# Chuanming-Liu/DAzimSurfTomo

Measured on AMD Instinct MI355X. Metric: FMM traveltime fields/sec (256^2 grid, 16 periods) + LSQR SpMV HBM GB/s, higher is better.
Workload: dtype f32

## Files before the change

### dazimsurftomo_amd/csrc/rays.hip

```cpp
#include <cmath>
#include <chrono>
#include <unistd.h>

#include "dazim_internal.h"

#include <rocprim/device/device_scan.hpp>
#include <rocprim/device/device_radix_sort.hpp>

namespace {

#ifdef DZ_RAYS_MARK
#define RAYS_MARK(i) asm volatile("; MARK " #i ::: "memory")
#else
#define RAYS_MARK(i)
#endif

constexpr int GDX = 5, GDZ = 5;
constexpr int RM = DAZIM_RMAX;
constexpr float EARTH = 6371.0f;
constexpr float FTOL = 1e-4f;

struct RayArgs {
  dazim_geom g;
  int nx, ny, nz, kmax;
  long nray;
  const int *field;
  const float *rcx, *rcz;
  const float *scx, *scz;
  const int *period;
  const int *kidx;
  const float *veln;
  const float *ttn;
  const int *tslot;
  int tsh;
  long fstride;
  const int *fdone;
  int *defer_mark;
  int max_quads;
  int sweeps;
  const float *ttnr;
  const int *nstsr;
  const dazim_refbox *boxes;
  const float *vels;
  const double *svs, *svp, *srho;
  unsigned nvx_magic;
  const double *skern;
  const float *lsen;
  double r_dnx, r_dnz, r_dnxr, r_dnzr, r_dvx, r_dvz, r_e2dnx, r_e2dnxr;
  float dplh;
  float *dsurf;
  int *status;
  int *rbflag;
  long *count;
  int *nlist;
  unsigned short *lcell;
  float *lval;
  float *fdm_scratch;
  int LK;
  int lcap;
  const unsigned *perm;
  unsigned *qcount;
  float2 *pts;
  int *npts;
  int pcap;
  int dense;
  long *countd;
  int plain_step;
  int keep_small;
  const long *rowptr;
  float *val;
  int *col;
};

__device__ __forceinline__ float dz_sinf(float x) {
  if (!(x > 0.0f && x < 3.1415927f)) return (float)sin((double)x);
  const double y = (double)x - 1.5707963267948966192;
  const double y2 = y * y;
  double p = -1.5619206968586226e-16;
  p = fma(p, y2, 4.7794773323873853e-14);
  p = fma(p, y2, -1.1470745597729725e-11);
  p = fma(p, y2, 2.0876756987868099e-09);
  p = fma(p, y2, -2.7557319223985891e-07);
  p = fma(p, y2, 2.4801587301587302e-05);
  p = fma(p, y2, -1.3888888888888889e-03);
  p = fma(p, y2, 4.1666666666666664e-02);
  p = fma(p, y2, -0.5);
  p = fma(p, y2, 1.0);
  return (float)p;
}

__device__ __forceinline__ void step_azimuth(float x0, float z0, float x1, float z1, float &c2psi, float &s2psi) {
  const float PI_F = 3.1415926535898f;
  const float evtlat = (PI_F / 2 - x0) * 180.0f / PI_F, evtlon = z0 * 180.0f / PI_F;
  const float stalat = (PI_F / 2 - x1) * 180.0f / PI_F, stalon = z1 * 180.0f / PI_F;
  const double pi = (double)3.1415926535898f;
  const float piby2 = (float)(pi / (double)2.f);
  const double rad = (double)2.f * pi / (double)360.f;
  const double sph = (double)(1.0f / 298.257f);
  const double scolat = (double)piby2 - atan((1. - sph) * (1. - sph) * tan((double)stalat * rad));
  const double ecolat = (double)piby2 - atan((1. - sph) * (1. - sph) * tan((double)evtlat * rad));
  const double slon = (double)stalon * rad, elon = (double)evtlon * rad;
  const double a = sin(scolat) * cos(slon), b = sin(scolat) * sin(slon), c = cos(scolat);
  const double dd = sin(elon), ee = -cos(elon), cc = cos(ecolat);
  const double gg = -cc * ee, hh = cc * dd, kk = -sin(ecolat);
  const double rhs1 = (a - dd) * (a - dd) + (b - ee) * (b - ee) + c * c - (double)2.f;
  const double rhs2 = (a - gg) * (a - gg) + (b - hh) * (b - hh) + (c - kk) * (c - kk) - (double)2.f;
  double daz = atan2(rhs1, rhs2);
  if (daz < 0.0) daz = daz + 2 * pi;
  float az = (float)(daz / rad);
  if (fabsf(az - 360.f) < .00001f) az = 0.0f;
  const float rgpsi = az / 180 * PI_F;
  c2psi = (float)cos((double)(2.0f * rgpsi));
  s2psi = (float)sin((double)(2.0f * rgpsi));
}

__device__ __forceinline__ float divr(float x, double rd) { return (float)((double)x * rd); }

__device__ __forceinline__ void basis(float v, float b[4]) {
  const float om = 1.0f - v;
  b[0] = om * om * om / 6.0f;
  b[1] = (4.0f - 6.0f * (v * v) + 3.0f * (v * v * v)) / 6.0f;
  b[2] = (1.0f + 3.0f * v + 3.0f * (v * v) - 3.0f * (v * v * v)) / 6.0f;
  b[3] = v * v * v / 6.0f;
}

__device__ __forceinline__ float div6(float x) { return divr(x, 1.0 / 6.0); }
__device__ __forceinline__ float basis1(float v, int i) {
  const float w = i == 0 ? 1.0f - v : v;
  const float t2 = w * w, t3 = t2 * w;
  const float p = i == 1 ? 4.0f : 1.0f + 3.0f * v;
  const float c = i == 1 ? -6.0f : 3.0f, d = i == 1 ? 3.0f : -3.0f;
  const float n = (p + c * t2) + d * t3;
  return div6((i == 0 || i == 3) ? t3 : n);
}

__device__ __forceinline__ float vel_at(const dazim_geom &g, const float *veln, int ipx, int ipz, float drx, float drz,
                                        double rdnx, double rdnz) {
  float vel = 0.0f;
#pragma unroll
  for (int l = 1; l <= 2; l++)
#pragma unroll
    for (int m = 1; m <= 2; m++) {
      float produ = (1.0f - fabsf(divr((float)(m - 1) * g.dnz - drz, rdnz)));
      produ = produ * (1.0f - fabsf(divr((float)(l - 1) * g.dnx - drx, rdnx)));
      if (ipz - 1 + m <= g.nnz && ipx - 1 + l <= g.nnx && ipz - 1 + m >= 1 && ipx - 1 + l >= 1)
        vel = vel + veln[(size_t)(ipx - 2 + l) * g.nnz + (ipz - 2 + m)] * produ;
    }
  return vel;
}
__device__ __forceinline__ float vel_at_interior(const dazim_geom &g, const float *veln, int ipx, int ipz, float drx, float drz,
                                                 double rdnx, double rdnz) {
  float vel = 0.0f;
#pragma unroll
  for (int l = 1; l <= 2; l++)
// ... 50 lines not shown
__device__ __forceinline__ void cbar() { asm volatile("" ::: "memory"); }

template <bool EMIT, bool AZIM, bool TILED, bool MAP>
__global__ __launch_bounds__(64, AZIM ? 2 : RAYS_MINW) void rays_kernel(RayArgs A_) {
  using ArgP = const __attribute__((address_space(4))) RayArgs *;
  auto launder = [](ArgP p) {
    int z;
    asm volatile("v_mov_b32 %0, 0" : "=v"(z));
    return (ArgP)((const __attribute__((address_space(4))) char *)p + __builtin_amdgcn_readfirstlane(z));
  };
  ArgP Ap = launder((ArgP)__builtin_amdgcn_kernarg_segment_ptr());
#define A (*Ap)
#define RAYS_ARGS_FRESH Ap = launder(Ap)
  constexpr int GP = EMIT ? GP_EMIT : GP_COUNT;
  constexpr int RPW = 64 / GP;
  constexpr int LPR = 16 / GP;
  constexpr int LSTEP = 4 / LPR;
  constexpr unsigned GMASK = (1u << GP) - 1u;
  extern __shared__ __attribute__((aligned(16))) unsigned short s_lists[];
  dazim_geom g;
  g.nvx = A.g.nvx; g.nvz = A.g.nvz; g.nnx = A.g.nnx; g.nnz = A.g.nnz;
  g.gox = A.g.gox; g.goz = A.g.goz; g.dnx = A.g.dnx; g.dnz = A.g.dnz; g.dvx = A.g.dvx; g.dvz = A.g.dvz;
  const int lane = threadIdx.x, grp = lane / GP, gl = lane & (GP - 1);
  const int lm = gl & 3, l0 = gl >> 2;
  const int nnx = g.nnx, nnz = g.nnz, nvx = g.nvx, nvz = g.nvz;
  const int ldf = nvx + 2, nf = ldf * (nvz + 2);
  constexpr int NG = AZIM ? 3 : 1;
  const unsigned nvx_magic = A.nvx_magic;
  const int LC = A.lcap;
  unsigned short *s_list = s_lists + (size_t)grp * LC;
  float *gfdm = A.fdm_scratch + ((size_t)blockIdx.x * RPW + grp) * nf * NG;
  float *gfdmc = gfdm + nf, *gfdms = gfdm + 2 * nf;
  __shared__ int s_rngs[RPW][4];
  int *s_rng = s_rngs[grp];
  constexpr int RC = 8;
  const float gox = g.gox, goz = g.goz, dnx = g.dnx, dnz = g.dnz, dvx = g.dvx, dvz = g.dvz;
  const double rdnx = A.r_dnx, rdnz = A.r_dnz, rdnxr = A.r_dnxr, rdnzr = A.r_dnzr, rdvx = A.r_dvx, rdvz = A.r_dvz;
  const unsigned gmask_shift = grp * GP;
  const long nquad = (A.nray + RPW - 1) / RPW;
  const int nxcd = (gridDim.x % 8 == 0) ? 8 : 1;
  unsigned *qcnt = A.qcount + (EMIT ? 8 : 0);
  int chunk = (int)(blockIdx.x % nxcd);
  int traced = 0;
  for (;;) {
    RAYS_ARGS_FRESH;
    long quad = -1;
    if (lane == 0) {
      for (int tried = 0; tried < nxcd; tried++) {
        const long lo = nquad * chunk / nxcd, hi = nquad * (chunk + 1) / nxcd;
        const long b = lo < hi ? (long)atomicAdd(&qcnt[chunk], 1u) : hi;
        if (lo + b < hi) {
          quad = lo + b;
          break;
        }
        if (!EMIT && A.sweeps > 1 && lo < hi && b < (hi - lo) * A.sweeps) {
          quad = lo + b % (hi - lo);
          break;
        }
        chunk = (chunk + 1) % nxcd;
      }
    }
    quad = ((long)__shfl((int)(quad >> 32), 0) << 32) | (unsigned)__shfl((int)quad, 0);
    chunk = __shfl(chunk, 0);
    if (quad < 0) break;
    const long slot = quad * RPW + grp;
    if (!EMIT && A.defer_mark) {
      if (!A.defer_mark[quad]) continue;
      if (A.fdone) {
        const int fq = slot < A.nray ? A.field[A.perm ? (long)A.perm[slot] : slot] : -1;
        const int st = fq >= 0 ? __hip_atomic_load(A.fdone + fq, __ATOMIC_ACQUIRE, __HIP_MEMORY_SCOPE_AGENT) : 1;
        if (__ballot(st != 1) != 0) continue;
        __builtin_amdgcn_fence(__ATOMIC_ACQUIRE, "agent");
      }
      if (A.max_quads > 0 && traced >= A.max_quads) break;
      int mine = 0;
      if (lane == 0) mine = __hip_atomic_exchange(A.defer_mark + quad, 0, __ATOMIC_RELAXED, __HIP_MEMORY_SCOPE_AGENT);
      mine = __shfl(mine, 0);
      if (!mine) continue;
      traced++;
      if (lane == 0) atomicAdd(&A.qcount[18], 1u);
    }
    if (slot >= A.nray) continue;
    const long ray = A.perm ? (long)A.perm[slot] : slot;
    const int f = A.field[ray];
    const float scx = A.scx[f], scz = A.scz[f], rcx = A.rcx[ray], rcz = A.rcz[ray];
    const float *veln = A.veln + (size_t)(A.period[f] - 1) * nnx * nnz;
    const float *ttn = TILED ? A.ttn + (size_t)(A.tslot ? A.tslot[f] : f) * A.fstride : A.ttn + (size_t)f * nnx * nnz;
    const int tsh = TILED ? A.tsh : 0;
    auto tnode = [&](int x0, int z0) -> float {
      return TILED ? ttn[dz_tile_x(x0, tsh) + dz_tile_z(z0)] : ttn[(size_t)x0 * nnz + z0];
    };
    const float *ttnr = A.ttnr + (size_t)f * RM * RM;
    const int *nstsr = A.nstsr + (size_t)f * RM * RM;
    const dazim_refbox bx = A.boxes[f];
    const int saved = EMIT ? A.nlist[ray] : -1;
    if (saved < 0 && gl < 4) s_rng[gl] = gl < 2 ? 0x7fffffff : -1;
    cbar();
    int status = 0, rb = 0;
    if (!EMIT) {
      int irx = (int)divr(rcx - gox, rdnx) + 1, irz = (int)divr(rcz - goz, rdnz) + 1;
      if (irx < 1 || irx > nnx || irz < 1 || irz > nnz) status = DAZIM_E_RECEIVER_OUTSIDE;
      if (!status) {
        if (irx == nnx) irx--;
        if (irz == nnz) irz--;
        const int isx = (int)divr(scx - gox, rdnx) + 1, isz = (int)divr(scz - goz, rdnz) + 1;
        float sred = ((scx - rcx) * EARTH) * ((scx - rcx) * EARTH);
        const float e2 = (scz - rcz) * EARTH * dz_sinf(rcx);
        sred = sqrtf(sred + e2 * e2);
        bool sw = sred < A.dplh;
        if (isx == irx && isz == irz) sw = true;
        float trr;
        if (sw) {
          const float vs = bilin_cell(g, veln, isx, isz, scx, scz, rdnx, rdnz);
          const float vr = bilin_cell(g, veln, irx, irz, rcx, rcz, rdnx, rdnz);
          trr = 2.0f * sred / (vs + vr);
        } else {
          const float drx = (rcx - gox) - (float)(irx - 1) * dnx;
          const float drz = (rcz - goz) - (float)(irz - 1) * dnz;
          trr = 0.0f;
#pragma unroll
          for (int k = 1; k <= 2; k++)
#pragma unroll
            for (int l = 1; l <= 2; l++) {
              const float produ = (1.0f - fabsf(divr((float)(l - 1) * dnz - drz, rdnz))) *
                                  (1.0f - fabsf(divr((float)(k - 1) * dnx - drx, rdnx)));
              trr = trr + tnode(irx - 2 + k, irz - 2 + l) * produ;
            }
        }
        if (gl == 0) A.dsurf[ray] = trr;
      }
    }
    const float goxr = bx.goxr, gozr = bx.gozr, dnxr = bx.dnxr, dnzr = bx.dnzr;
    const int nnxr = bx.nnxr, nnzr = bx.nnzr;
    const int isx = (int)divr(scx - goxr, rdnxr) + 1, isz = (int)divr(scz - gozr, rdnzr) + 1;
    const float dpl = 0.5f * A.dplh;
    int ipx = (int)divr(rcx - gox, rdnx) + 1, ipz = (int)divr(rcz - goz, rdnz) + 1;
    if (ipx < 1 || ipx >= nnx || ipz < 1 || ipz >= nnz) status = DAZIM_E_RECEIVER_OUTSIDE;
    if (!status && saved < 0) {
      float x0 = rcx, z0 = rcz;
      float sinx0 = dz_sinf(x0);
      int sw = 0;
      float sred = ((scx - x0) * EARTH) * ((scx - x0) * EARTH);
      float e2 = (scz - z0) * EARTH * sinx0;
      sred = sqrtf(sred + e2 * e2);
      if (sred < 2.0f * dpl) sw = 1;
      int ipxr = (int)divr(rcx - goxr, rdnxr) + 1, ipzr = (int)divr(rcz - gozr, rdnzr) + 1;
      auto in_refined = [&](int px, int pz) -> int {
        if (px < 1 || px >= nnxr || pz < 1 || pz >= nnzr) return 0;
        const int *sp = nstsr + (size_t)(px - 1) * RM + (pz - 1);
        if (sp[0] != 0 || sp[1] != 0) return 0;
        if (sp[RM] != 0 || sp[RM + 1] != 0) return 0;
        return 1;
      };
      int igref = in_refined(ipxr, ipzr);
      if (sw == 0 && igref == 1 && ipxr == isx && ipzr == isz) sw = 1;
      const bool keep_pts = !EMIT && A.pts != nullptr && gl == 0;
      float2 *rp = A.pts ? A.pts + (size_t)ray * A.pcap : nullptr;
      int np = 1;
      if (keep_pts) {
        rp[0] = make_float2(rcx, rcz);
        if (sw == 1) { if (A.pcap > 1) rp[1] = make_float2(scx, scz); np = 2; }
      }
      int cbx = -100, cbz = -100;
      float acc[LPR], accc[LPR], accs[LPR];
#pragma unroll
      for (int q = 0; q < LPR; q++) acc[q] = accc[q] = accs[q] = 0.0f;
// ... 351 lines not shown
          float rowv = 0.0f;
          int nn = 0;
          bool cell = li < ntot;
          int c = 0;
          if (cell) c = lovf ? li : s_list[li];
          const int jj = (int)__umulhi((unsigned)c, nvx_magic) + 1, kk = c - (jj - 1) * nvx + 1;
          if (cell && lovf) cell = fabsf(gfdm[jj * ldf + kk]) >= FTOL;
          if (cell && MAP) {
            rowv = (blk == 0 ? gfdm : (blk == 1 ? gfdmc : gfdms))[jj * ldf + kk];
            keep = A.keep_small ? (rowv != 0.0f) : (fabsf(rowv) > FTOL);
            nn = blk * bstride + poff + (jj - 1) * nvx + kk;
          } else if (cell) {
            const size_t si = ((size_t)(k - 1) * A.kmax + kslot) * ncol + (size_t)jj * (nvx + 2) + kk;
            if (blk == 0) {
              const float fd = gfdm[jj * ldf + kk];
              double r;
              if (A.skern) {
                r = A.skern[si] * (double)fd;
              } else {
                const float v = A.vels[((size_t)(k - 1) * A.ny + jj) * A.nx + kk];
                const float coe_a = (2.0947f - 0.8206f * 2 * v + 0.2683f * 3 * (v * v) - 0.0251f * 4 * (v * v * v));
                const float vpft = 0.9409f + 2.0947f * v - 0.8206f * (v * v) + 0.2683f * (v * v * v) - 0.0251f * (v * v * v * v);
                const float coe_rho = coe_a * (1.6612f - 0.4721f * 2 * vpft + 0.0671f * 3 * (vpft * vpft) -
                                               0.0043f * 4 * (vpft * vpft * vpft) + 0.000106f * 5 * (vpft * vpft * vpft * vpft));
                r = (A.svp[si] * (double)coe_a + A.srho[si] * (double)coe_rho + A.svs[si]) * (double)fd;
              }
              rowv = (float)r;
              if (A.dense) {
                const float vL = A.vels[((size_t)(k - 1) * A.ny + jjL) * A.nx + kkL];
                const float caL = (2.0947f - 0.8206f * 2 * vL + 0.2683f * 3 * (vL * vL) - 0.0251f * 4 * (vL * vL * vL));
                const float vpL = 0.9409f + 2.0947f * vL - 0.8206f * (vL * vL) + 0.2683f * (vL * vL * vL) - 0.0251f * (vL * vL * vL * vL);
                const float crL = caL * (1.6612f - 0.4721f * 2 * vpL + 0.0671f * 3 * (vpL * vpL) -
                                         0.0043f * 4 * (vpL * vpL * vpL) + 0.000106f * 5 * (vpL * vpL * vpL * vpL));
                const double rd = (A.svp[si] * (double)caL + A.srho[si] * (double)crL + A.svs[si]) * (double)fd;
                keepd = (float)rd != 0.0f;
                if (EMIT && A.dense == 1) rowv = (float)rd;
              }
            } else {
              rowv = A.lsen[si] * (blk == 1 ? gfdmc : gfdms)[jj * ldf + kk];
              keepd = rowv != 0.0f;
            }
            keep = A.keep_small ? (rowv != 0.0f) : (fabsf(rowv) > FTOL);
            if (EMIT && A.dense == 1) keep = keepd;
            nn = blk * bstride + (k - 1) * nvz * nvx + (jj - 1) * nvx + kk;
          }
          if (!EMIT && A.dense == 2) cntd += __popc((unsigned)((__ballot(keepd) >> gmask_shift) & GMASK));
          const unsigned m = (unsigned)((__ballot(keep) >> gmask_shift) & GMASK);
          if (EMIT && keep) {
            const long pos = rstart + cnt + __popc(m & ((1u << gl) - 1u));
            A.val[pos] = rowv;
            A.col[pos] = nn - 1;
          }
          cnt += __popc(m);
        }
      }
    cbar();
    if (saved < 0) {
      const int x0 = max(s_rng[0], 0), x1 = min(s_rng[2] + 3, nvx + 1), z0 = max(s_rng[1], 0), z1 = min(s_rng[3] + 3, nvz + 1);
      for (int z = z0; z <= z1; z++)
        for (int x = x0 + gl; x <= x1; x += GP) {
          gfdm[z * ldf + x] = 0.0f;
          if (AZIM) { gfdmc[z * ldf + x] = 0.0f; gfdms[z * ldf + x] = 0.0f; }
        }
    } else if (!rowcache) {
      for (int i = gl; i < nlist; i += GP) {
        const int c = s_list[i];
        const int jj = (int)__umulhi((unsigned)c, nvx_magic) + 1, kk = c - (jj - 1) * nvx + 1;
        gfdm[jj * ldf + kk] = 0.0f;
        if (AZIM) { gfdmc[jj * ldf + kk] = 0.0f; gfdms[jj * ldf + kk] = 0.0f; }
      }
    }
    cbar();
    if (!EMIT && gl == 0) {
      A.count[ray] = cnt;
      if (A.dense == 2) A.countd[ray] = cntd;
      if (lovf) atomicAdd(&A.qcount[16], 1u);
      if (!status && nlist > A.LK) atomicAdd(&A.qcount[17], 1u);
    }
  }
}
#undef A
#undef RAYS_ARGS_FRESH

struct RayBuild {
  dazim_ctx *ctx;
  int nx = 0, ny = 0, nz = 0, kmax = 0, nfield = 0;
  float goxd = 0, gozd = 0, dvxd = 0, dvzd = 0;
  const float *vels = nullptr, *scx = nullptr, *scz = nullptr, *veln = nullptr, *ttn = nullptr, *ttnr = nullptr, *rcx = nullptr, *rcz = nullptr;
  const float *lsen = nullptr;
  const int *period = nullptr, *kidx = nullptr, *nstsr = nullptr, *field = nullptr;
  const dazim_refbox *boxes = nullptr;
  const double *svs = nullptr, *svp = nullptr, *srho = nullptr;
  int64_t nray = 0;
  float *dsurf = nullptr;
  dazim_csr **G = nullptr;
  int64_t *nnz_out = nullptr;
  int *n_boundary = nullptr;
  bool map = false, azim = false;
  struct StreamSwap {
    dazim_ctx *c; hipStream_t main; bool on = false;
    void restore() { if (on) { c->stream = main; on = false; } }
    ~StreamSwap() {
      if (on) (void)hipStreamSynchronize(c->stream);
      restore();
    }
  } swap;
  struct {
    DzBuf<float> vels, scx, scz, veln, ttn, ttnr, rcx, rcz, dsurf, lsen;
    DzBuf<int> period, kidx, nstsr, field;
    DzBuf<dazim_refbox> boxes;
    DzBuf<double> svs, svp, srho;
  } d;
  struct Arrays {
    dazim_ctx *c; int64_t *rp = nullptr; float *v = nullptr; int *cl = nullptr; int64_t nnz = 0, cap_nnz = 0; bool keep = false;
    ~Arrays() { if (!keep) { dz_big_put(c, rp); dz_big_put(c, v); dz_big_put(c, cl); } }
  } arrays, arrays_d;
  dazim_geom g;
  bool joint = false, tiled = false, overlap = false, twin = false;
  size_t nn = 0, nr = 0, ncol = 0, nk = 0, nr1 = 0, lds = 0;
  int64_t res_rows = 0, res_nnz = 0;
  long nwg = 0;
  double overlap_tail_s = 0.0;
  RayArgs A;
  explicit RayBuild(dazim_ctx *c) : ctx(c), swap{c, c ? c->stream : nullptr}, arrays{c}, arrays_d{c} {}
  int check() {
    if (!ctx || !G) return DAZIM_E_BAD_ARG;
    joint = map ? azim : lsen != nullptr;
    if (map) nz = 2;
    if (map && dz_opt(ctx, "rays.dense_twin", 0) != 0)
      return dz_fail(ctx, DAZIM_E_BAD_ARG, "dazim_rays_build_G_maps: option rays.dense_twin serves the 3-D program's diagnostics only");
    if (dazim_geometry(nx, ny, goxd, gozd, dvxd, dvzd, &g)) return dz_fail(ctx, DAZIM_E_BAD_ARG, "bad grid");
    if (nray < 0 || nfield < 1 || nz < 2 || kmax < 1 || (size_t)g.nvx * g.nvz > 65535u) return dz_fail(ctx, DAZIM_E_BAD_ARG, "bad arguments to dazim_rays_build_G");
    tiled = ttn == nullptr;
    if (tiled && (!ctx->fields.tiled || ctx->fields.nfield != nfield || ctx->fields.nnx != g.nnx || ctx->fields.nnz != g.nnz))
      return dz_fail(ctx, DAZIM_E_BAD_ARG, "dazim_rays_build_G: ttn is NULL and the last dazim_fmm_batch call did not keep %d fields of this grid inside the library (call it with ttn = NULL)", nfield);
    if (!scx || !scz || !period || !veln || !ttnr || !nstsr || !boxes || !dsurf ||
        (!map && (!vels || !svs || !svp || !srho)) || (nray > 0 && (!field || !rcx || !rcz)))
      return dz_fail(ctx, DAZIM_E_BAD_ARG, "dazim_rays_build_G: NULL array (the refined fields ttnr, nstsr and boxes of dazim_fmm_batch are required)");
    DZ_HIP(hipSetDevice(ctx->device));
    return 0;
  }
  int decide_overlap() {
    overlap = (bool)ctx->fmm_finish && tiled && ctx->fields.fdone && nray > 0;
    if (overlap && ctx->aux_epilogue && ctx->comm && ((DzComm *)ctx->comm)->nccl) overlap = false;
    if (overlap)
      for (const void *q : {(const void *)vels, (const void *)scx, (const void *)scz, (const void *)period, (const void *)veln,
                            (const void *)ttnr, (const void *)nstsr, (const void *)boxes, (const void *)field, (const void *)rcx,
                            (const void *)rcz, (const void *)svs, (const void *)svp, (const void *)srho, (const void *)dsurf,
                            (const void *)kidx, (const void *)lsen})
        if (q && !dz_is_device_ptr(q)) overlap = false;
    if (!overlap) { const int rcf = dz_fmm_finish(ctx); if (rcf) return rcf; }
    if (overlap) {
      DZ_HIP(hipStreamWaitEvent(ctx->stream3, ctx->ev_pre, 0));
      ctx->stream = ctx->stream3;
      swap.on = true;
    }
    return dz_join_aux(ctx);
  }
  int stage_inputs() {
    nn = (size_t)g.nnx * g.nnz; nr = (size_t)RM * RM; ncol = (size_t)nx * ny;
    int rc;
    if (!map && (rc = d.vels.init(ctx, vels, (size_t)nz * ncol, true, false))) return rc;
    if ((rc = d.scx.init(ctx, scx, nfield, true, false)) || (rc = d.scz.init(ctx, scz, nfield, true, false)) ||
        (rc = d.period.init(ctx, period, nfield, true, false)) || (rc = d.kidx.init(ctx, kidx ? kidx : period, nfield, true, false)) ||
        (rc = d.veln.init(ctx, veln, nn * kmax, true, false)) || (!tiled && (rc = d.ttn.init(ctx, ttn, nn * nfield, true, false))) ||
        (rc = d.ttnr.init(ctx, ttnr, nr * nfield, true, false)) || (rc = d.nstsr.init(ctx, nstsr, nr * nfield, true, false)) ||
        (rc = d.boxes.init(ctx, boxes, nfield, true, false)) || (rc = d.field.init(ctx, field, nray, true, false)) ||
        (rc = d.rcx.init(ctx, rcx, nray, true, false)) || (rc = d.rcz.init(ctx, rcz, nray, true, false)))
      return rc;
    nk = (size_t)nz * kmax * ncol;
    if (!map && ((rc = d.svs.init(ctx, svs, nk, true, false)) || (rc = d.svp.init(ctx, svp, nk, true, false)) ||
                  (rc = d.srho.init(ctx, srho, nk, true, false))))
      return rc;
    if ((rc = d.dsurf.init(ctx, dsurf, nray, false, true))) return rc;
    if (joint && !map && (rc = d.lsen.init(ctx, lsen, (size_t)(nz - 1) * kmax * ncol, true, false))) return rc;
    if ((rc = dz_check_range(ctx, d.period.dev, nfield, 1, kmax, "period_idx"))) return rc;
    if ((rc = dz_check_range(ctx, d.kidx.dev, nfield, 1, kmax, "kernel_idx"))) return rc;
    return dz_check_range(ctx, d.field.dev, nray, 0, nfield - 1, "field_of_ray");
  }
  int kernel_constants() {
    int rc;
    A.g = g;
    A.nx = nx; A.ny = ny; A.nz = nz; A.kmax = kmax;
    A.nray = nray;
    A.field = d.field.dev; A.rcx = d.rcx.dev; A.rcz = d.rcz.dev; A.scx = d.scx.dev; A.scz = d.scz.dev;
    A.period = d.period.dev; A.kidx = d.kidx.dev; A.veln = d.veln.dev; A.ttn = d.ttn.dev; A.ttnr = d.ttnr.dev;
    A.tslot = nullptr; A.tsh = 0; A.fstride = (long)nn;
    if (tiled) {
      A.ttn = reinterpret_cast<const float *>(ctx->fields.tiled);
      A.tslot = ctx->fields.tslot; A.tsh = ctx->fields.tsh; A.fstride = ctx->fields.stride;
    }
    ctx->ksec["rays.tiled_fields"] = tiled ? 1.0 : 0.0;
    ctx->ksec["rays.map"] = map ? 1.0 : 0.0;
    ctx->ksec["rays.overlap"] = overlap ? 1.0 : 0.0;
    A.fdone = overlap ? ctx->fields.fdone : nullptr;
    A.defer_mark = nullptr; A.max_quads = 0; A.sweeps = 1;
    A.nstsr = d.nstsr.dev; A.boxes = d.boxes.dev; A.vels = d.vels.dev; A.svs = d.svs.dev; A.svp = d.svp.dev; A.srho = d.srho.dev;
    A.lsen = joint && !map ? d.lsen.dev : nullptr;
    A.skern = nullptr;
    {
      const unsigned dv = (unsigned)g.nvx;
      A.nvx_magic = (unsigned)((0x100000000ull + dv - 1) / dv);
      for (unsigned c = 0; c < 65536u; c++)
        if ((unsigned)(((unsigned long long)c * A.nvx_magic) >> 32) != c / dv) return dz_fail(ctx, DAZIM_E_BAD_ARG, "internal: reciprocal of nvx");
    }
    if (!map && dz_opt(ctx, "rays.skern", 1) != 0) {
      double *pk;
      if ((rc = dz_scratch(ctx, "rays.skern", nk, &pk))) return rc;
      hipLaunchKernelGGL(k_row_kernels, dim3((unsigned)((nk + 255) / 256)), dim3(256), 0, ctx->stream, (long)nk, kmax, (long)ncol,
                         d.vels.dev, d.svs.dev, d.svp.dev, d.srho.dev, pk);
      DZ_HIP(hipGetLastError());
      A.skern = pk;
    }
    {
      float dpl = g.dnx * EARTH;
      float rd1 = g.dnz * EARTH * sinf(g.gox);
      if (rd1 < dpl) dpl = rd1;
      rd1 = g.dnz * EARTH * sinf(g.gox + (float)(g.nnx - 1) * g.dnx);
      if (rd1 < dpl) dpl = rd1;
      A.dplh = dpl;
    }
    {
      const float dnxr = g.dvx / (float)(GDX * 8), dnzr = g.dvz / (float)(GDZ * 8);
      const float e2dnx = 2.0f * EARTH * g.dnx, e2dnxr = 2.0f * EARTH * dnxr;
      A.r_dnx = 1.0 / (double)g.dnx;   A.r_dnz = 1.0 / (double)g.dnz;
      A.r_dnxr = 1.0 / (double)dnxr;   A.r_dnzr = 1.0 / (double)dnzr;
      A.r_dvx = 1.0 / (double)g.dvx;   A.r_dvz = 1.0 / (double)g.dvz;
      A.r_e2dnx = 1.0 / (double)e2dnx; A.r_e2dnxr = 1.0 / (double)e2dnxr;
    }
    return 0;
  }
  int scratch() {
    int rc;
    nr1 = (size_t)(nray > 0 ? nray : 1);
    if ((rc = dz_scratch(ctx, "rays.status", nr1, &A.status))) return rc;
    if ((rc = dz_scratch(ctx, "rays.rb", nr1, &A.rbflag))) return rc;
    if ((rc = dz_scratch(ctx, "rays.count", (size_t)(nray + 1), &A.count))) return rc;
    A.lcap = g.nvx * g.nvz <= 4096 ? 512 : 1024;
    if (dz_opt(ctx, "rays.lcap", 0) >= 16 && dz_opt(ctx, "rays.lcap", 0) <= 8192) A.lcap = dz_opt(ctx, "rays.lcap", 0);
    if (A.lcap > g.nvx * g.nvz) A.lcap = g.nvx * g.nvz;
    A.LK = A.lcap;
    A.keep_small = dz_opt(ctx, "rays.keep_small", 0) != 0 ? 1 : 0;
    A.plain_step = dz_opt(ctx, "rays.plain_step", 0) != 0 ? 1 : 0;
    A.pts = nullptr; A.npts = nullptr; A.pcap = 0;
    if (dz_opt(ctx, "rays.keep_paths", 0) != 0) {
      A.pcap = 4 * (g.nnx + g.nnz) + 16;
      if ((rc = dz_scratch(ctx, "rays.pts", nr1 * (size_t)A.pcap, &A.pts))) return rc;
      if ((rc = dz_scratch(ctx, "rays.npts", nr1, &A.npts))) return rc;
      DZ_HIP(hipMemsetAsync(A.npts, 0, nr1 * 4, ctx->stream));
    }
    ctx->ksec["rays.path_cap"] = A.pcap;
    ctx->ksec["rays.path_rays"] = A.pts ? (double)nray : 0.0;
    twin = dz_opt(ctx, "rays.dense_twin", 0) != 0 && !A.keep_small;
    A.dense = twin ? 2 : 0;
    A.countd = nullptr;
    if (twin) {
      if ((rc = dz_scratch(ctx, "rays.countd", (size_t)(nray + 1), &A.countd))) return rc;
      DZ_HIP(hipMemsetAsync(A.countd, 0, (size_t)(nray + 1) * 8, ctx->stream));
    }
    if ((rc = dz_scratch(ctx, "rays.nlist", nr1, &A.nlist))) return rc;
    if ((rc = dz_scratch(ctx, "rays.lcell", nr1 * A.LK, &A.lcell))) return rc;
    if ((rc = dz_scratch(ctx, "rays.lval", nr1 * A.LK * (joint ? 3 : 1), &A.lval))) return rc;
    res_rows = (int64_t)g.nvx * g.nvz * (map ? kmax : nz - 1) * (joint ? 3 : 1);
    res_nnz = (map ? 5 : 7) * res_rows;
    if (dz_opt(ctx, "csr.reserve_rows", 0) > res_rows) res_rows = dz_opt(ctx, "csr.reserve_rows", 0);
    if (dz_opt(ctx, "csr.reserve_nnz", 0) > res_nnz) res_nnz = dz_opt(ctx, "csr.reserve_nnz", 0);
    if ((rc = dz_big_get(ctx, (size_t)(nray + res_rows + 1), &arrays.rp))) return rc;
    A.dsurf = d.dsurf.dev;
    A.rowptr = (const long *)arrays.rp; A.val = nullptr; A.col = nullptr;
    return 0;
  }
  template <int I> static const void *kernel_no() { return (const void *)rays_kernel<(I & 8) != 0, (I & 4) != 0, (I & 2) != 0, (I & 1) != 0>; }
  const void *kern(bool emit) const {
    static const void *const tab[16] = {kernel_no<0>(),  kernel_no<1>(),  kernel_no<2>(),  kernel_no<3>(), kernel_no<4>(),  kernel_no<5>(),
                                        kernel_no<6>(),  kernel_no<7>(),  kernel_no<8>(),  kernel_no<9>(), kernel_no<10>(), kernel_no<11>(),
                                        kernel_no<12>(), kernel_no<13>(), kernel_no<14>(), kernel_no<15>()};
    return tab[(emit ? 8 : 0) + (joint ? 4 : 0) + (tiled ? 2 : 0) + (map ? 1 : 0)];
  }
  int launch(bool emit, const RayArgs &R, long nwg_) {
    RayArgs args = R;
    void *params[] = {&args};
    DZ_HIP(hipLaunchKernel(kern(emit), dim3((unsigned)nwg_), dim3(64), params, lds, ctx->stream));
    return 0;
  }
  int launch_shape() {
    lds = (size_t)A.lcap * 2 * RPW_MAX + 16;
    DZ_HIP(hipFuncSetAttribute(kern(false), hipFuncAttributeMaxDynamicSharedMemorySize, (int)lds));
    DZ_HIP(hipFuncSetAttribute(kern(true), hipFuncAttributeMaxDynamicSharedMemorySize, (int)lds));
    int per_cu = (int)(160 * 1024 / (lds + 256));
    {
      int occ = 0;
      const void *kf = kern(false);
      if (hipOccupancyMaxActiveBlocksPerMultiprocessor(&occ, kf, 64, lds) == hipSuccess && occ > 0 && occ < per_cu) per_cu = occ;
    }
    if (per_cu > 16) per_cu = 16;
    if (per_cu < 1) return dz_fail(ctx, DAZIM_E_BAD_ARG, "inversion grid too large for the LDS cell lists");
    if (dz_opt(ctx, "rays.wg_per_cu", 0) > 0 && dz_opt(ctx, "rays.wg_per_cu", 0) < per_cu) per_cu = dz_opt(ctx, "rays.wg_per_cu", 0);
    nwg = (long)ctx->num_cu * per_cu;
    if (nwg > (nray + RPW_MAX - 1) / RPW_MAX) nwg = (nray + RPW_MAX - 1) / RPW_MAX;
    if (dz_opt(ctx, "rays.nwg", 0) > 0 && dz_opt(ctx, "rays.nwg", 0) < nwg) nwg = dz_opt(ctx, "rays.nwg", 0);
    if (nwg >= 8) nwg -= nwg % 8;
    if (nwg < 1) nwg = 1;
    const size_t nslot = (size_t)nwg * RPW_MAX * (g.nvx + 2) * (g.nvz + 2) * (joint ? 3 : 1);
    int rc;
    if ((rc = dz_scratch(ctx, "rays.fdm", nslot, &A.fdm_scratch))) return rc;
    DZ_HIP(hipMemsetAsync(A.fdm_scratch, 0, nslot * sizeof(float), ctx->stream));
    ctx->ksec["rays.nwg"] = (double)nwg;
    return 0;
  }
  int sort_rays() {
    int rc;
    A.perm = nullptr;
    if (nray >= 64 && nray < (1ll << 32) && dz_opt(ctx, "rays.sort", 1) != 0) {
      int fbits = 1;
      while ((1ll << fbits) < nfield) fbits++;
      const int dbits = 32 - fbits > 12 ? 12 : 32 - fbits;
      if (dbits >= 4) {
        unsigned *k0, *k1, *v0, *v1;
        if ((rc = dz_scratch(ctx, "rays.sortbuf", (size_t)nray * 4 + 16, &k0))) return rc;
        k1 = k0 + nray; v0 = k1 + nray; v1 = v0 + nray;
        const float ex = (float)g.nnx * g.dnx, ez = (float)g.nnz * g.dnz;
        const float inv_dmax = 1.0f / sqrtf(ex * ex + ez * ez);
        hipLaunchKernelGGL(k_ray_keys, dim3((unsigned)((nray + 255) / 256)), dim3(256), 0, ctx->stream, (long)nray, d.field.dev, d.scx.dev,
                           d.scz.dev, d.rcx.dev, d.rcz.dev, inv_dmax, dbits, k0, v0, overlap ? A.tslot : (const int *)nullptr);
        size_t tb = 0;
        DZ_HIP(rocprim::radix_sort_pairs(nullptr, tb, k0, k1, v0, v1, (size_t)nray, 0, fbits + dbits, ctx->stream));
        void *tmp;
        if ((rc = dz_scratch(ctx, "rays.sorttmp", tb + 256, &tmp))) return rc;
        DZ_HIP(rocprim::radix_sort_pairs(tmp, tb, k0, k1, v0, v1, (size_t)nray, 0, fbits + dbits, ctx->stream));
        A.perm = v1;
      }
    }
    if ((rc = dz_scratch(ctx, "rays.qcount", 32, &A.qcount))) return rc;
    DZ_HIP(hipMemsetAsync(A.qcount, 0, 128, ctx->stream));
    if (overlap) {
      const size_t nq = (size_t)((nray + RPW_MAX - 1) / RPW_MAX) + 8;
      if ((rc = dz_scratch(ctx, "rays.defer", nq, &A.defer_mark))) return rc;
      DZ_HIP(hipMemsetAsync(A.defer_mark, 0, nq * 4, ctx->stream));
    }
    return 0;
  }
  int count_pass() { return nray > 0 ? launch(false, A, nwg) : 0; }
  int count_passes_beside_eikonal() {
    int rc;
    const auto t_poll0 = std::chrono::steady_clock::now();
    auto fmm_over = [&]() {
      const bool over = hipEventQuery(ctx->ev_f1) == hipSuccess;
      if (!over) (void)hipGetLastError();
      return over;
    };
    if (ctx->fields.hprog && ctx->fields.total_tasks > 0) {
      const unsigned slack = ctx->fields.nwg / 4 + 8 * 16;
      const unsigned total = ctx->fields.total_tasks;
      const unsigned want = total > slack ? total - slack : 0;
      for (;;) {
        unsigned have = 0;
        for (int c = 0; c < 8; c++) have += ctx->fields.hprog[c];
        if (have >= want || fmm_over()) break;
        if (std::chrono::steady_clock::now() - t_poll0 > std::chrono::seconds(120)) break;
        usleep(50);
      }
    }
    const unsigned nquad_all = (unsigned)((nray + RPW_MAX - 1) / RPW_MAX);
    unsigned pending = nquad_all, *h_traced = nullptr;
    { void *hp; if ((rc = dz_pinned(ctx, "rays.host_pending", 64, &hp))) return rc; h_traced = (unsigned *)hp; }
    DZ_HIP(hipMemsetAsync(A.defer_mark, 1, (size_t)nquad_all * 4, ctx->stream));
    int npass = 0;
    bool collected = false, ev0_set = false;
    unsigned left_by_first = 0;
    int rcf = 0;
    while (pending > 0) {
      const bool last = fmm_over();
      if (last && !collected) {
        swap.restore();
        DZ_HIP(hipStreamSynchronize(ctx->stream3));
        rcf = dz_fmm_finish(ctx);
        collected = true;
        if (rcf) break;
        if (npass == 0) (void)hipEventRecord(ctx->ev_r1, ctx->stream);
        (void)hipEventRecord(ctx->ev0, ctx->stream);
        ev0_set = true;
      }
      long nwg_pass = nwg;
      A.max_quads = 0;
      A.sweeps = collected ? 1 : 3;
      if (collected) A.fdone = nullptr;
      DZ_HIP(hipMemsetAsync(A.qcount, 0, 32, ctx->stream));
      if ((rc = launch(false, A, nwg_pass))) return rc;
      if (!collected) DZ_HIP(hipEventRecord(ctx->ev_r1, ctx->stream));
      DZ_HIP(hipMemcpyAsync(h_traced, A.qcount + 18, 4, hipMemcpyDeviceToHost, ctx->stream));
      DZ_HIP(hipStreamSynchronize(ctx->stream));
      const unsigned before = pending;
      pending = collected ? 0u : nquad_all - *h_traced;
      if (npass == 0) left_by_first = pending;
      npass++;
      if (pending > 0 && pending == before) usleep(100);
    }
    swap.restore();
    if (!collected) rcf = dz_fmm_finish(ctx);
    DZ_HIP(hipStreamSynchronize(ctx->stream3));
    if (rcf) return rcf;
    ctx->ksec["rays.passes"] = npass;
    ctx->ksec["rays.deferred_quads"] = left_by_first;
    A.fdone = nullptr; A.defer_mark = nullptr; A.max_quads = 0; A.sweeps = 1;
    float ms_tail = 0;
    if (hipEventElapsedTime(&ms_tail, ctx->ev_f1, ctx->ev_r1) == hipSuccess && ms_tail > 0) overlap_tail_s = ms_tail * 1e-3;
    if (!ev0_set) (void)hipEventRecord(ctx->ev0, ctx->stream);
    return 0;
  }
  int scan_and_emit(Arrays &M, long *count, int64_t slack, bool dense_twin) {
    int rc; void *p; size_t tb = 0;
    DZ_HIP(rocprim::exclusive_scan(nullptr, tb, count, (long *)M.rp, 0l, (size_t)(nray + 1), rocprim::plus<long>(), ctx->stream));
    if ((rc = dz_scratch(ctx, "rays.scan", tb + 256, &p))) return rc;
    DZ_HIP(rocprim::exclusive_scan(p, tb, count, (long *)M.rp, 0l, (size_t)(nray + 1), rocprim::plus<long>(), ctx->stream));
    DZ_HIP(hipMemcpyAsync(&M.nnz, M.rp + nray, 8, hipMemcpyDeviceToHost, ctx->stream));
    DZ_HIP(hipStreamSynchronize(ctx->stream));
    M.cap_nnz = M.nnz + slack;
    const size_t cap = (size_t)(M.cap_nnz > 0 ? M.cap_nnz : 1);
    if ((rc = dz_big_get(ctx, cap, &M.v)) || (rc = dz_big_get(ctx, cap, &M.cl))) return rc;
    RayArgs R = A;
    R.rowptr = (const long *)M.rp; R.val = M.v; R.col = M.cl;
    if (dense_twin) {
      R.dense = 1;
      DZ_HIP(hipMemsetAsync(A.qcount + 8, 0, 32, ctx->stream));
    }
    return nray > 0 ? launch(true, R, nwg) : 0;
  }
  int statuses() {
    int rc;
    std::vector<int> hs(nr1), hb(nr1);
    unsigned hq[2] = {0, 0};
    if (nray > 0) {
      DZ_HIP(hipMemcpyAsync(hq, A.qcount + 16, 8, hipMemcpyDeviceToHost, ctx->stream));
      DZ_HIP(hipMemcpyAsync(hs.data(), A.status, nray * 4, hipMemcpyDeviceToHost, ctx->stream));
      DZ_HIP(hipMemcpyAsync(hb.data(), A.rbflag, nray * 4, hipMemcpyDeviceToHost, ctx->stream));
      DZ_HIP(hipStreamSynchronize(ctx->stream));
    }
    int nb = 0, err = 0;
    for (int64_t i = 0; i < nray; i++) {
      nb += hb[i];
      if (hs[i] && !err) err = dz_fail(ctx, hs[i], "ray %ld: receiver lies outside model", (long)i);
    }
    if (n_boundary) *n_boundary = nb;
    if (nnz_out) *nnz_out = arrays.nnz;
    ctx->ksec["rays.list_sweeps"] = hq[0];
    ctx->ksec["rays.list_retraced"] = hq[1];
    ctx->ksec["rays.lcap"] = A.lcap;
    if ((rc = d.dsurf.finish())) return rc;
    DZ_HIP(hipStreamSynchronize(ctx->stream));
    return err;
  }
  int adopt() {
    int rc;
    const int64_t n = (int64_t)g.nvx * g.nvz * (map ? kmax : nz - 1) * (joint ? 3 : 1);
    arrays.keep = true;
    if ((rc = dz_csr_adopt_cap(ctx, nray, n, arrays.nnz, arrays.rp, arrays.cl, arrays.v, nray + res_rows, arrays.cap_nnz, G))) return rc;
    if (twin) {
      dazim_csr *Gd = nullptr;
      arrays_d.keep = true;
      if ((rc = dz_csr_adopt_cap(ctx, nray, n, arrays_d.nnz, arrays_d.rp, arrays_d.cl, arrays_d.v, 0, 0, &Gd)) || (rc = dz_csr_set_twin(ctx, *G, Gd))) {
        dazim_csr_free(ctx, *G);
        *G = nullptr;
        return rc;
      }
    }
    return 0;
  }
  int run() {
    int rc;
    if ((rc = check()) || (rc = decide_overlap()) || (rc = stage_inputs()) || (rc = kernel_constants()) || (rc = scratch()) ||
        (rc = launch_shape()) || (rc = sort_rays()))
      return rc;
    DzTimer t(ctx, "rays");
    DZ_HIP(hipMemsetAsync(A.count, 0, (size_t)(nray + 1) * 8, ctx->stream));
    if ((rc = overlap ? count_passes_beside_eikonal() : count_pass())) return rc;
    if ((rc = scan_and_emit(arrays, A.count, res_nnz, false))) return rc;
    if (twin && ((rc = dz_big_get(ctx, (size_t)(nray + 1), &arrays_d.rp)) || (rc = scan_and_emit(arrays_d, A.countd, 0, true)))) return rc;
    t.stop();
    if (overlap) {
      ctx->ksec["rays.after_fmm_count"] = overlap_tail_s;
      ctx->ksec["rays"] += overlap_tail_s;
    }
    return (rc = statuses()) ? rc : adopt();
  }
};

}

extern "C" int dazim_rays_build_G(dazim_ctx *ctx, int nx, int ny, int nz, float goxd, float gozd, float dvxd,
                                  float dvzd, int kmax, const float *vels, int nfield, const float *scx,
                                  const float *scz, const int *period, const int *kidx, const float *veln,
                                  const float *ttn, const float *ttnr, const int *nstsr, const dazim_refbox *boxes,
                                  int64_t nray, const int *field, const float *rcx, const float *rcz,
                                  const double *svs, const double *svp, const double *srho, float *dsurf,
                                  dazim_csr **G, int64_t *nnz_out, int *n_boundary) {
  RayBuild b(ctx);
  b.nx = nx; b.ny = ny; b.nz = nz; b.goxd = goxd; b.gozd = gozd; b.dvxd = dvxd; b.dvzd = dvzd;
  b.kmax = kmax; b.vels = vels; b.svs = svs; b.svp = svp; b.srho = srho;
  b.nfield = nfield; b.scx = scx; b.scz = scz; b.period = period; b.kidx = kidx;
  b.veln = veln; b.ttn = ttn; b.ttnr = ttnr; b.nstsr = nstsr; b.boxes = boxes;
  b.nray = nray; b.field = field; b.rcx = rcx; b.rcz = rcz;
  b.dsurf = dsurf; b.G = G; b.nnz_out = nnz_out; b.n_boundary = n_boundary;
  return b.run();
}
extern "C" int dazim_rays_build_G_joint(dazim_ctx *ctx, int nx, int ny, int nz, float goxd, float gozd, float dvxd,
                                        float dvzd, int kmax, const float *vels, int nfield, const float *scx,
                                        const float *scz, const int *period, const int *kidx, const float *veln,
                                        const float *ttn, const float *ttnr, const int *nstsr,
                                        const dazim_refbox *boxes, int64_t nray, const int *field, const float *rcx,
                                        const float *rcz, const double *svs, const double *svp, const double *srho,
                                        const float *lsen, float *dsurf, dazim_csr **G, int64_t *nnz_out,
                                        int *n_boundary) {
  if (!lsen) return dz_fail(ctx, DAZIM_E_BAD_ARG, "joint mode needs Lsen_Gsc");
  RayBuild b(ctx);
  b.nx = nx; b.ny = ny; b.nz = nz; b.goxd = goxd; b.gozd = gozd; b.dvxd = dvxd; b.dvzd = dvzd;
  b.kmax = kmax; b.vels = vels; b.svs = svs; b.svp = svp; b.srho = srho; b.lsen = lsen;
  b.nfield = nfield; b.scx = scx; b.scz = scz; b.period = period; b.kidx = kidx;
  b.veln = veln; b.ttn = ttn; b.ttnr = ttnr; b.nstsr = nstsr; b.boxes = boxes;
  b.nray = nray; b.field = field; b.rcx = rcx; b.rcz = rcz;
  b.dsurf = dsurf; b.G = G; b.nnz_out = nnz_out; b.n_boundary = n_boundary;
  return b.run();
}

extern "C" int dazim_rays_build_G_maps(dazim_ctx *ctx, int nx, int ny, float goxd, float gozd, float dvxd, float dvzd, int kmax,
                                       int azim, int nfield, const float *scx, const float *scz, const int *period,
                                       const float *veln, const float *ttn, const float *ttnr, const int *nstsr,
                                       const dazim_refbox *boxes, int64_t nray, const int *field, const float *rcx,
                                       const float *rcz, float *dsurf, dazim_csr **G, int64_t *nnz_out, int *n_boundary) {
  RayBuild b(ctx);
// ... 30 lines not shown
```

Baseline: 56440.

## Emit CSR rows directly from saved cell lists instead of re-tracing rays

Adds a wave-per-ray emit kernel that builds CSR values and columns from the per-ray cell lists saved during the count pass, multiplying them by the sensitivity kernels with prefetched layer blocks. The full tracing kernel then runs in emit mode only for rays whose lists overflowed, and skips rays that already have a saved list. This removes a second full ray trace in the common case, at the cost of an extra host readback of the overflow counter and a second kernel launch when some rays overflowed.

```diff
diff --git a/dazimsurftomo_amd/csrc/rays.hip b/dazimsurftomo_amd/csrc/rays.hip
--- a/dazimsurftomo_amd/csrc/rays.hip
+++ b/dazimsurftomo_amd/csrc/rays.hip
@@ -70,6 +70,7 @@
   const long *rowptr;
   float *val;
   int *col;
+  int skip_saved;
 };
 
 __device__ __forceinline__ float dz_sinf(float x) {
@@ -286,6 +287,7 @@
     }
     if (slot >= A.nray) continue;
     const long ray = A.perm ? (long)A.perm[slot] : slot;
+    if (EMIT && A.skip_saved && A.nlist[ray] >= 0) continue;
     const int f = A.field[ray];
     const float scx = A.scx[f], scz = A.scz[f], rcx = A.rcx[ray], rcz = A.rcz[ray];
     const float *veln = A.veln + (size_t)(A.period[f] - 1) * nnx * nnz;
@@ -803,6 +805,150 @@
 #undef A
 #undef RAYS_ARGS_FRESH
 
+
+template <int NIT, bool MAP, typename T>
+__device__ __forceinline__ void emit_block(const T *__restrict__ tab, size_t kstep, int nlay, int nk0, int ncell, int n, int lane,
+                                           const int (&cid)[NIT], const int (&sidx)[NIT], const float (&fdv)[NIT], bool keep_small,
+                                           float *__restrict__ val, int *__restrict__ col, long rstart, long rend, int &cnt) {
+  constexpr int KB = 4;
+  T cur[KB][NIT], nxt[KB][NIT];
+  auto load = [&](T (&d)[KB][NIT], int k0) {
+#pragma unroll
+    for (int q = 0; q < KB; q++)
+#pragma unroll
+      for (int i = 0; i < NIT; i++) d[q][i] = MAP ? (T)0 : tab[(size_t)(min(k0 + q, nlay) - 1) * kstep + sidx[i]];
+  };
+  load(nxt, 1);
+  for (int k0 = 1; k0 <= nlay; k0 += KB) {
+#pragma unroll
+    for (int q = 0; q < KB; q++)
+#pragma unroll
+      for (int i = 0; i < NIT; i++) cur[q][i] = nxt[q][i];
+    load(nxt, k0 + KB);
+#pragma unroll
+    for (int q = 0; q < KB; q++) {
+      if (k0 + q > nlay) break;
+      const int nk = nk0 + (k0 + q - 1) * ncell;
+#pragma unroll
+      for (int i = 0; i < NIT; i++) {
+        float rowv;
+        if (MAP) rowv = fdv[i];
+        else if (sizeof(T) == 8) rowv = (float)(cur[q][i] * (double)fdv[i]);
+        else rowv = (float)cur[q][i] * fdv[i];
+        const bool keep = i * 64 + lane < n && (keep_small ? (rowv != 0.0f) : (fabsf(rowv) > FTOL));
+        const unsigned long long m = __ballot(keep);
+        const long pos = rstart + cnt + (int)__builtin_amdgcn_mbcnt_hi((unsigned)(m >> 32), __builtin_amdgcn_mbcnt_lo((unsigned)m, 0u));
+        if (keep && pos < rend) {
+          val[pos] = rowv;
+          col[pos] = nk + cid[i];
+        }
+        cnt += __popcll(m);
+      }
+    }
+  }
+}
+
+template <int NIT, bool AZIM, bool MAP>
+__device__ __forceinline__ void emit_row(const RayArgs &A, int lane, int n, const int (&c01)[2], const float (&f01)[2],
+                                         const unsigned short *__restrict__ lc, const float *__restrict__ lv, const double *__restrict__ skern,
+                                         const float *__restrict__ lsen, float *__restrict__ val, int *__restrict__ col, size_t sk0,
+                                         size_t kstep, int poff, int bstride, int nlay, long rstart, long rend) {
+  constexpr int NG = AZIM ? 3 : 1;
+  constexpr int NR = NIT > 0 ? NIT : 1;
+  const int nvx = A.g.nvx, ncell = nvx * A.g.nvz;
+  const unsigned nvx_magic = A.nvx_magic;
+  const bool keep_small = A.keep_small != 0;
+  auto decode = [&](int li, int craw, int &c, int &si) {
+    c = li < n ? craw : 0;
+    const int jj = (int)__umulhi((unsigned)c, nvx_magic) + 1, kk = c - (jj - 1) * nvx + 1;
+    si = jj * (nvx + 2) + kk;
+  };
+  int cnt = 0;
+  if (NIT > 0) {
+    int cid[NR], sidx[NR];
+    float fdv[NR];
+#pragma unroll
+    for (int i = 0; i < NR; i++) decode(i * 64 + lane, c01[i], cid[i], sidx[i]);
+#pragma unroll
+    for (int blk = 0; blk < NG; blk++) {
+#pragma unroll
+      for (int i = 0; i < NR; i++) fdv[i] = i * 64 + lane < n ? (blk == 0 ? f01[i] : lv[(size_t)blk * A.LK + i * 64 + lane]) : 0.0f;
+      const int nk0 = blk * bstride + poff;
+      if (blk == 0) emit_block<NR, MAP, double>(MAP ? nullptr : skern + sk0, kstep, nlay, nk0, ncell, n, lane, cid, sidx, fdv, keep_small, val, col, rstart, rend, cnt);
+      else emit_block<NR, MAP, float>(MAP ? nullptr : lsen + sk0, kstep, nlay, nk0, ncell, n, lane, cid, sidx, fdv, keep_small, val, col, rstart, rend, cnt);
+    }
+    return;
+  }
+  const int nit = (n + 63) >> 6;
+  for (int blk = 0; blk < NG; blk++) {
+    const float *__restrict__ ls = lv + (size_t)blk * A.LK;
+    for (int k = 1; k <= nlay; k++) {
+      const size_t sk = sk0 + (size_t)(k - 1) * kstep;
+      const int nk = blk * bstride + poff + (k - 1) * ncell;
+      for (int it = 0; it < nit; it++) {
+        const int li = it * 64 + lane;
+        int c, si;
+        decode(li, li < n ? (int)lc[li] : 0, c, si);
+        float rowv = 0.0f;
+        bool keep = false;
+        if (li < n) {
+          const float fd = ls[li];
+          if (MAP) rowv = fd;
+          else if (blk == 0) rowv = (float)(skern[sk + si] * (double)fd);
+          else rowv = lsen[sk + si] * fd;
+          keep = keep_small ? (rowv != 0.0f) : (fabsf(rowv) > FTOL);
+        }
+        const unsigned long long m = __ballot(keep);
+        const long pos = rstart + cnt + (int)__builtin_amdgcn_mbcnt_hi((unsigned)(m >> 32), __builtin_amdgcn_mbcnt_lo((unsigned)m, 0u));
+        if (keep && pos < rend) {
+          val[pos] = rowv;
+          col[pos] = nk + c;
+        }
+        cnt += __popcll(m);
+      }
+    }
+  }
+}
+
+constexpr int ER_WAVES = 4;
+template <bool AZIM, bool MAP>
+__global__ __launch_bounds__(64 * ER_WAVES) void emit_rows_kernel(RayArgs A) {
+  constexpr int NG = AZIM ? 3 : 1;
+  const int lane = threadIdx.x & 63, wave = __builtin_amdgcn_readfirstlane((int)(threadIdx.x >> 6));
+  auto uni = [](int v) { return __builtin_amdgcn_readfirstlane(v); };
+  auto unil = [&](long v) { return ((long)uni((int)(v >> 32)) << 32) | (unsigned)uni((int)v); };
+  const size_t ncol = (size_t)A.nx * A.ny;
+  const int ncell = A.g.nvx * A.g.nvz;
+  const int nlay = MAP ? 1 : A.nz - 1;
+  const int bstride = MAP ? A.kmax * ncell : ncell * (A.nz - 1);
+  const size_t kstep = (size_t)A.kmax * ncol;
+  const long stride = (long)gridDim.x * ER_WAVES;
+  for (long ray = (long)blockIdx.x * ER_WAVES + wave; ray < A.nray; ray += stride) {
+    const unsigned short *lc = A.lcell + (size_t)ray * A.LK;
+    const float *lv = A.lval + (size_t)ray * NG * A.LK;
+    int nv = A.nlist[ray], fv = A.field[ray];
+    long r0 = A.rowptr[ray], r1 = A.rowptr[ray + 1];
+    int c01[2];
+    float f01[2];
+#pragma unroll
+    for (int i = 0; i < 2; i++) {
+      const int li = min(i * 64 + lane, A.LK - 1);
+      c01[i] = lc[li];
+      f01[i] = lv[li];
+    }
+    asm volatile("" : "+v"(nv), "+v"(fv), "+v"(r0), "+v"(r1), "+v"(c01[0]), "+v"(c01[1]), "+v"(f01[0]), "+v"(f01[1]));
+    const int n = uni(nv);
+    if (n <= 0) continue;
+    const int f = uni(fv);
+    const size_t sk0 = MAP ? 0 : (size_t)(uni(A.kidx[f]) - 1) * ncol;
+    const int poff = MAP ? (uni(A.period[f]) - 1) * ncell : 0;
+    const long rstart = unil(r0), rend = unil(r1);
+    if (n <= 64) emit_row<1, AZIM, MAP>(A, lane, n, c01, f01, lc, lv, A.skern, A.lsen, A.val, A.col, sk0, kstep, poff, bstride, nlay, rstart, rend);
+    else if (n <= 128) emit_row<2, AZIM, MAP>(A, lane, n, c01, f01, lc, lv, A.skern, A.lsen, A.val, A.col, sk0, kstep, poff, bstride, nlay, rstart, rend);
+    else emit_row<0, AZIM, MAP>(A, lane, n, c01, f01, lc, lv, A.skern, A.lsen, A.val, A.col, sk0, kstep, poff, bstride, nlay, rstart, rend);
+  }
+}
+
 struct RayBuild {
   dazim_ctx *ctx;
   int nx = 0, ny = 0, nz = 0, kmax = 0, nfield = 0;
@@ -842,6 +988,7 @@
   int64_t res_rows = 0, res_nnz = 0;
   long nwg = 0;
   double overlap_tail_s = 0.0;
+  int64_t rows_emitted = 0;
   RayArgs A;
   explicit RayBuild(dazim_ctx *c) : ctx(c), swap{c, c ? c->stream : nullptr}, arrays{c}, arrays_d{c} {}
   int check() {
@@ -989,6 +1136,7 @@
     if ((rc = dz_big_get(ctx, (size_t)(nray + res_rows + 1), &arrays.rp))) return rc;
     A.dsurf = d.dsurf.dev;
     A.rowptr = (const long *)arrays.rp; A.val = nullptr; A.col = nullptr;
+    A.skip_saved = 0;
     return 0;
   }
   template <int I> static const void *kernel_no() { return (const void *)rays_kernel<(I & 8) != 0, (I & 4) != 0, (I & 2) != 0, (I & 1) != 0>; }
@@ -1002,6 +1150,16 @@
     RayArgs args = R;
     void *params[] = {&args};
     DZ_HIP(hipLaunchKernel(kern(emit), dim3((unsigned)nwg_), dim3(64), params, lds, ctx->stream));
+    return 0;
+  }
+  int launch_rows(const RayArgs &R) {
+    static const void *const tab[4] = {(const void *)emit_rows_kernel<false, false>, (const void *)emit_rows_kernel<false, true>,
+                                       (const void *)emit_rows_kernel<true, false>, (const void *)emit_rows_kernel<true, true>};
+    long nblk = (long)((nray + ER_WAVES - 1) / ER_WAVES);
+    if (nblk > (1l << 24)) nblk = 1l << 24;
+    RayArgs args = R;
+    void *params[] = {&args};
+    DZ_HIP(hipLaunchKernel(tab[(joint ? 2 : 0) + (map ? 1 : 0)], dim3((unsigned)nblk), dim3(64 * ER_WAVES), params, 0, ctx->stream));
     return 0;
   }
   int launch_shape() {
@@ -1134,7 +1292,9 @@
     DZ_HIP(rocprim::exclusive_scan(nullptr, tb, count, (long *)M.rp, 0l, (size_t)(nray + 1), rocprim::plus<long>(), ctx->stream));
     if ((rc = dz_scratch(ctx, "rays.scan", tb + 256, &p))) return rc;
     DZ_HIP(rocprim::exclusive_scan(p, tb, count, (long *)M.rp, 0l, (size_t)(nray + 1), rocprim::plus<long>(), ctx->stream));
+    unsigned retraced = 0;
     DZ_HIP(hipMemcpyAsync(&M.nnz, M.rp + nray, 8, hipMemcpyDeviceToHost, ctx->stream));
+    DZ_HIP(hipMemcpyAsync(&retraced, A.qcount + 17, 4, hipMemcpyDeviceToHost, ctx->stream));
     DZ_HIP(hipStreamSynchronize(ctx->stream));
     M.cap_nnz = M.nnz + slack;
     const size_t cap = (size_t)(M.cap_nnz > 0 ? M.cap_nnz : 1);
@@ -1145,7 +1305,15 @@
       R.dense = 1;
       DZ_HIP(hipMemsetAsync(A.qcount + 8, 0, 32, ctx->stream));
     }
-    return nray > 0 ? launch(true, R, nwg) : 0;
+    if (nray <= 0) return 0;
+    const bool rows = !twin && (map || A.skern != nullptr) && dz_opt(ctx, "rays.emit_rows", 1) != 0;
+    if (rows) {
+      if ((rc = launch_rows(R))) return rc;
+      R.skip_saved = 1;
+      rows_emitted = nray - (int64_t)retraced;
+      if (retraced == 0) return 0;
+    }
+    return launch(true, R, nwg);
   }
   int statuses() {
     int rc;
@@ -1166,6 +1334,7 @@
     if (nnz_out) *nnz_out = arrays.nnz;
     ctx->ksec["rays.list_sweeps"] = hq[0];
     ctx->ksec["rays.list_retraced"] = hq[1];
+    ctx->ksec["rays.emit_rows"] = (double)rows_emitted;
     ctx->ksec["rays.lcap"] = A.lcap;
     if ((rc = d.dsurf.finish())) return rc;
     DZ_HIP(hipStreamSynchronize(ctx->stream));
```

Result: no change. 56870, median of 6 (+0.8%).
